# mandt-lab/PSLD

Hardware: AMD Instinct MI355X
Metric: train images/sec, CIFAR-10 PSLD (6ch 32x32) NCSN++ HSM step (higher is better)
Workload: dtype f32

## Files before the change

psld_amd/csrc/conv_wino.hip:

```cpp
#include <cstdlib>
#include <cstring>
#include <type_traits>

#include "common.h"
#include "psld_hip.h"
#include "tile_shared.h"
#include "limb.h"

namespace {

constexpr int WT = 32;
constexpr int VPLANE = WT * ROWB;
constexpr int VBYTES = 16 * 3 * VPLANE;
constexpr int WINO_THREADS = 512;

struct WinoArgs {
    const float* x1;
    const float* x2;
    int C1, C2;
    int B, H, W;
    const u32x4* ufrag;
    int N, M;
    int chunks;
    float* C;
// ... 111 lines not shown
        int lo = 0, hi = ntab - 1;
        while (lo < hi) {
            const int mid = (lo + hi + 1) >> 1;
            if (tab[8 * mid + 7] <= idx) lo = mid; else hi = mid - 1;
        }
        const long long* d = tab + 8 * lo;
        wino_pack_item<NL>(reinterpret_cast<const float*>(d[0]), reinterpret_cast<u32x4*>(d[1]), idx - d[7], (int)d[3], d[5], d[6],
                       (int)d[4]);
    }
}

template <int ABL = 0, bool GNF = false, bool ERAW = false, int LA = 2, bool TAIL = false, int NL = 3, bool SH = false>
__global__ void __launch_bounds__(WINO_THREADS) wino_conv8s_kernel(const WinoArgs a) {
    extern __shared__ __attribute__((aligned(16))) unsigned char smem[];
    constexpr int NI = 4;
    constexpr int RAWB = NI * 64 * 128;
    unsigned char* Vs = smem;
    unsigned char* Rs = smem + VBYTES / 3 * NL;

    const int tid = threadIdx.x;
    const int lane = tid & 63, wave = __builtin_amdgcn_readfirstlane(tid >> 6);
    const int tiles_n = TAIL ? (a.N + 127) >> 7 : a.N >> 7;
    const int nsp = a.ksplit > 1 ? a.ksplit : 1;
    const int tiles_m = a.tiles_m;
    const int per_range = tiles_m * tiles_n;
    const int vb = xcd_remap(blockIdx.x, gridDim.x);
    const int split = nsp > 1 ? vb / per_range : 0;
    const int bid = vb - split * per_range;
    const int kch = a.chunks >> a.lg_ksplit, ch0 = split * kch;
    float* const Cw = a.C + split * a.slab_stride;
    const int tile_n = a.nmajor ? bid / tiles_m : bid % tiles_n;
    const int tile_m = a.nmajor ? bid - tile_n * tiles_m : bid / tiles_n;
    const int n0 = tile_n * 128;
    const bool live = !TAIL || n0 + wave * 16 < a.N;

    const int HW = a.H * a.W;
    const int W2 = a.cw + 2;
    const int lg_tx = a.lg_tiles_x, lg_tps = a.lg_tps;
    const int rpi = HW >= 128 ? HW >> 7 : 1;
    const int tm_img = a.lg_rpi >= 0 ? tile_m >> a.lg_rpi : tile_m / rpi;
    const int reg = tile_m - tm_img * rpi;
    const int img0 = HW >= 128 ? tm_img : tile_m * a.nseg;
    const int oy0 = (reg >> a.lg_xblocks) * a.rps, ox0 = (reg & ((1 << a.lg_xblocks) - 1)) * a.cw;
    const float* zp = a.zero;

    const int c4 = tid & 7;
    int hoff[NI], rdst[NI];
    {
        const int seg_px = (a.rps + 2) * W2;
#pragma unroll
        for (int i = 0; i < NI; ++i) {
            const int px = (tid + WINO_THREADS * i) >> 3;
            const int seg = wino_div16(px, a.mul_seg);
            const int rem = px - seg * seg_px;
            const int hr = wino_div16(rem, a.mul_w2), hx = rem - hr * W2;
            const int img = img0 + seg, iy = oy0 + hr - 1, ix = ox0 + hx - 1;
            const bool ok = seg < a.nseg && img < a.B && iy >= 0 && iy < a.H && ix >= 0 && ix < a.W;
            hoff[i] = ok ? (img * a.H + iy) * a.W + ix : -1;
            rdst[i] = raw_off(px, c4);
        }
    }
    f32x4 hv[NI];
    auto load_raw = [&](int c) {
        const int c0 = c * 32;
        const bool second = c0 >= a.C1;
        const float* src = second ? a.x2 : a.x1;
        const int cs = second ? a.C2 : a.C1;
// ... 53 lines not shown
#pragma unroll
        for (int c = 0; c < 4; ++c) {
            ea[c] = *reinterpret_cast<const f32x4*>(Rb + t_ro[ra_ - v_r][c]);
            eb[c] = *reinterpret_cast<const f32x4*>(Rb + t_ro[rb_ - v_r][c]);
        }
        f32x4 r[4];
#pragma unroll
        for (int c = 0; c < 4; ++c) r[c] = plus ? ea[c] + eb[c] : ea[c] - eb[c];
#pragma unroll
        for (int j = 0; j < 4; ++j) {
            const f32x4 v = j == 0 ? r[0] - r[2] : j == 1 ? r[1] + r[2] : j == 2 ? r[2] - r[1] : r[1] - r[3];
            unsigned h0, m0_, l0, h1, m1, l1;
            if constexpr (NL == 3) {
                split3(v[0], v[1], h0, m0_, l0);
                split3(v[2], v[3], h1, m1, l1);
            } else if constexpr (NL == 2) {
                split2(v[0], v[1], h0, m0_);
                split2(v[2], v[3], h1, m1);
            } else if constexpr (SH) {
                h0 = cvt_pk_f16(v[0] * a.opscale, v[1] * a.opscale);
                h1 = cvt_pk_f16(v[2] * a.opscale, v[3] * a.opscale);
            } else {
                h0 = cvt_pk_f16(v[0], v[1]);
                h1 = cvt_pk_f16(v[2], v[3]);
            }
            unsigned char* q = Vs + (vrow * 4 + j) * NL * VPLANE + t_dst;
            *reinterpret_cast<u32x2*>(q) = u32x2{h0, h1};
            if constexpr (NL >= 2) *reinterpret_cast<u32x2*>(q + VPLANE) = u32x2{m0_, m1};
            if constexpr (NL == 3) *reinterpret_cast<u32x2*>(q + 2 * VPLANE) = u32x2{l0, l1};
        }
    };

    const int r16 = lane & 15, kq = lane >> 4;
    int aoff[2];
#pragma unroll
    for (int tb = 0; tb < 2; ++tb) {
        const int row = tb * 16 + r16;
        aoff[tb] = row * ROWB + ((kq ^ lds_swz(row)) << 4);
    }
    const u32x4* ub = a.ufrag + ((long long)(tile_n * 8 + ((ABL & 128) ? (wave & 3) : wave)) * a.chunks + ch0) * (16 * NL * 64);
    u32x4 bq[4][NL];
    auto load_b = [&](int sigma, u32x4 (&dst)[NL]) {
        const u32x4* p = ub + (long long)sigma * (NL * 64);
#pragma unroll
        for (int l = 0; l < NL; ++l) dst[l] = p[l * 64 + lane];
    };
    f32x4v acc[16][2];
#pragma unroll
    for (int p = 0; p < 16; ++p)
#pragma unroll
        for (int tb = 0; tb < 2; ++tb) acc[p][tb] = f32x4v{0.f, 0.f, 0.f, 0.f};
    u32x4 fa[NL == 1 ? 2 : NL][2];
    auto read_a = [&](int p, int l) {
#pragma unroll
        for (int tb = 0; tb < 2; ++tb) fa[l][tb] = *reinterpret_cast<const u32x4*>(Vs + (p * NL + l) * VPLANE + aoff[tb]);
    };
    auto mm = [&](int p, int la, int lb) {
#pragma unroll
        for (int tb = 0; tb < 2; ++tb) {
            if constexpr (NL == 1)
                acc[p][tb] = __builtin_amdgcn_mfma_f32_16x16x32_f16(
                    __builtin_bit_cast(f16x8, bq[p & 3][lb]), __builtin_bit_cast(f16x8, fa[la][tb]), acc[p][tb], 0, 0, 0);
            else
                acc[p][tb] = __builtin_amdgcn_mfma_f32_16x16x32_bf16(
                    __builtin_bit_cast(bf16x8, bq[p & 3][lb]), __builtin_bit_cast(bf16x8, fa[la][tb]), acc[p][tb], 0, 0, 0);
        }
    };
    auto mfma_half = [&](auto HH, auto LAST, int c) {
        constexpr int h = decltype(HH)::value;
        constexpr bool last = decltype(LAST)::value;
        if constexpr ((ABL & 256) != 0) __builtin_amdgcn_s_setprio(2);
        if constexpr (NL == 1) {
            auto read_a1 = [&](int p) {
#pragma unroll
                for (int tb = 0; tb < 2; ++tb) fa[p & 1][tb] = *reinterpret_cast<const u32x4*>(Vs + p * VPLANE + aoff[tb]);
            };
            read_a1(8 * h);
#pragma unroll
            for (int i = 0; i < 8; ++i) {
                const int p = 8 * h + i;
                if (!(last && p + LA >= 16)) load_b(c * 16 + p + LA, bq[(p + LA) & 3]);
                if (i < 7) read_a1(p + 1);
                __builtin_amdgcn_sched_barrier(0);
                mm(p, p & 1, 0);
                __builtin_amdgcn_sched_barrier(0);
            }
            return;
        }
        if constexpr (NL == 3) read_a(8 * h, 2);
        if constexpr (NL >= 2) read_a(8 * h, 1);
        read_a(8 * h, 0);
#pragma unroll
        for (int i = 0; i < 8; ++i) {
            const int p = 8 * h + i;
            if (!(ABL & 2) && !(last && p + LA >= 16)) load_b(c * 16 + p + LA, bq[(p + LA) & 3]);
            __builtin_amdgcn_sched_barrier(0);
            if constexpr (NL == 3) {
                mm(p, 2, 0);
                __builtin_amdgcn_sched_barrier(0);
                if (i < 7) read_a(p + 1, 2);
                __builtin_amdgcn_sched_barrier(0);
                mm(p, 1, 1);
            }
            if constexpr (NL >= 2) {
                mm(p, 1, 0);
                __builtin_amdgcn_sched_barrier(0);
                if (i < 7) read_a(p + 1, 1);
                __builtin_amdgcn_sched_barrier(0);
            }
            if constexpr (NL == 3) mm(p, 0, 2);
            if constexpr (NL >= 2) mm(p, 0, 1);
            mm(p, 0, 0);
            __builtin_amdgcn_sched_barrier(0);
            if (i < 7) read_a(p + 1, 0);
        }
        if constexpr ((ABL & 256) != 0) __builtin_amdgcn_s_setprio(0);
    };
    using I0 = std::integral_constant<int, 0>;
    using I1 = std::integral_constant<int, 1>;
    if constexpr ((ABL & 4) == 0 && (ABL & 256) == 0) { if (vr != 0) __builtin_amdgcn_s_setprio(1); }

    load_raw(ch0);
    if (live) {
        load_b(0, bq[0]);
        load_b(1, bq[1]);
        if (LA > 2) load_b(2, bq[2]);
    }
    store_raw(0, ch0);
    if constexpr (ERAW) load_raw(ch0 + min(1, kch - 1));
    __syncthreads();
    if (vr == 0) transform(I0{}, I0{}, 0); else transform(I0{}, I1{}, 0);
    __syncthreads();

    auto stamp = [&](int c, int idx) {
        if constexpr ((ABL & 64) != 0) {
            if (c == 3 && a.dbg) {
                __builtin_amdgcn_sched_barrier(0);
                const unsigned long long t = __builtin_amdgcn_s_memtime();
                if (lane == 0) a.dbg[((long long)blockIdx.x * 8 + wave) * 8 + idx] = t;
                __builtin_amdgcn_sched_barrier(0);
            }
        }
    };
    using No = std::false_type;
    using Yes = std::true_type;

    for (int c = 0; c < kch - 1; ++c) {
        stamp(c, 0);
        if constexpr (!ERAW) load_raw(ch0 + c + 1);
        if (vr == 0 && !(ABL & 1)) transform(I1{}, I0{}, c & 1);
        __builtin_amdgcn_sched_barrier(0);
        if (vr == 0) stamp(c, 1);
        if (live) mfma_half(I0{}, No{}, c);
        __builtin_amdgcn_sched_barrier(0);
        if (vr != 0) stamp(c, 1);
        if (vr != 0 && !(ABL & 1)) transform(I1{}, I1{}, c & 1);
        stamp(c, 2);
        store_raw((c + 1) & 1, ch0 + c + 1);
        stamp(c, 3);
// ... 4 lines not shown
        if (vr == 0) stamp(c, 5);
        if (live) mfma_half(I1{}, No{}, c);
        __builtin_amdgcn_sched_barrier(0);
        if (vr != 0) stamp(c, 5);
        if constexpr (ERAW) load_raw(ch0 + min(c + 2, kch - 1));
        if (vr != 0 && !(ABL & 1)) transform(I0{}, I1{}, (c + 1) & 1);
        stamp(c, 6);
        __syncthreads();
        stamp(c, 7);
    }
    {
        int c = kch - 1;
        asm volatile("" : "+s"(c));
        stamp(c, 0);
        if (vr == 0 && !(ABL & 1)) transform(I1{}, I0{}, c & 1);
        __builtin_amdgcn_sched_barrier(0);
        if (vr == 0) stamp(c, 1);
        if (live) mfma_half(I0{}, No{}, c);
        __builtin_amdgcn_sched_barrier(0);
        if (vr != 0) stamp(c, 1);
        if (vr != 0 && !(ABL & 1)) transform(I1{}, I1{}, c & 1);
        stamp(c, 2);
        stamp(c, 3);
        __syncthreads();
        stamp(c, 4);
        __builtin_amdgcn_sched_barrier(0);
        stamp(c, 5);
        if (live) mfma_half(I1{}, Yes{}, c);
        __builtin_amdgcn_sched_barrier(0);
        stamp(c, 6);
        stamp(c, 7);
    }

    if (!live) return;
    const PsldEpilogue& e = a.e;
    const int cn = n0 + wave * 16 + 4 * kq;
    const int org = (img0 * a.H + oy0) * a.W + ox0;
    const f32x4v zero4 = {0.f, 0.f, 0.f, 0.f};
    const bool rb_div = e.rowbias && !a.rb_img;
    char* const c_b = reinterpret_cast<char*>(Cw + (long long)org * a.ldc);
    const char* const res_b = reinterpret_cast<const char*>(e.res ? e.res + (long long)org * e.ldres : zp);
    f32x4v epi_bias, epi_tbv[2], epi_rv[2][4], epi_cv[2][4];
    int epi_rel[2];
    bool epi_ok[2];
    auto epi_rows = [&](auto TB) {
        constexpr int tb = decltype(TB)::value;
#pragma unroll
        for (int j = 0; j < 4; ++j) {
            const int px = epi_rel[tb] + (j >> 1) * a.W + (j & 1);
            epi_rv[tb][j] = e.res ? *reinterpret_cast<const f32x4v*>(res_b + (unsigned)((px * e.ldres + cn) * 4)) : zero4;
            epi_cv[tb][j] = e.accumulate ? *reinterpret_cast<const f32x4v*>(c_b + (unsigned)((px * a.ldc + cn) * 4)) : zero4;
        }
    };
    auto epi_request = [&]() {
        epi_bias = e.bias ? *reinterpret_cast<const f32x4v*>(e.bias + cn) : zero4;
#pragma unroll
        for (int tb = 0; tb < 2; ++tb) {
            const int tile = tb * 16 + r16;
            const int seg = tile >> lg_tps, rem = tile & ((1 << lg_tps) - 1);
            const int ty = rem >> lg_tx, tx = rem & ((1 << lg_tx) - 1);
            epi_ok[tb] = img0 + seg < a.B;
            epi_rel[tb] = epi_ok[tb] ? seg * HW + 2 * ty * a.W + 2 * tx : 0;
            epi_tbv[tb] = a.rb_img ? *reinterpret_cast<const f32x4v*>(
                                         e.rowbias + (long long)(epi_ok[tb] ? img0 + seg : img0) * e.ld_rowbias + cn)
                                   : zero4;
        }
        epi_rows(I0{});
    };
    epi_request();
    epi_rows(I1{});
    const f32x4v bias4 = epi_bias;
#pragma unroll
    for (int tb = 0; tb < 2; ++tb) {
        const bool ok = epi_ok[tb];
        const int rel = epi_rel[tb];
#pragma unroll
        for (int i = 0; i < 4; ++i) {
            const f32x4v s0 = (acc[4 * i][tb] + acc[4 * i + 1][tb]) + acc[4 * i + 2][tb];
            acc[4 * i + 1][tb] = (acc[4 * i + 1][tb] - acc[4 * i + 2][tb]) - acc[4 * i + 3][tb];
            acc[4 * i][tb] = s0;
        }
        const f32x4v add4 = bias4 + epi_tbv[tb];
        f32x4v o[2][2];
#pragma unroll
        for (int ya = 0; ya < 2; ++ya)
#pragma unroll
            for (int xb = 0; xb < 2; ++xb) {
                const f32x4v y = ya == 0 ? (acc[xb][tb] + acc[4 + xb][tb]) + acc[8 + xb][tb]
                                         : (acc[4 + xb][tb] - acc[8 + xb][tb]) - acc[12 + xb][tb];
                f32x4v addv = add4;
                if (rb_div)
                    addv = bias4 + *reinterpret_cast<const f32x4v*>(
                                       e.rowbias + (long long)((org + rel + ya * a.W + xb) / e.rows_per_img) * e.ld_rowbias + cn);
                f32x4v x = y * e.alpha + addv;
                if (e.res) x += epi_rv[tb][ya * 2 + xb];
                x *= e.out_scale;
                if (e.accumulate) x += epi_cv[tb][ya * 2 + xb];
                o[ya][xb] = x;
            }
        const bool gn_on = e.gn_part != nullptr;
        double gs = 0.0, gss = 0.0;
        if (ok) {
#pragma unroll
            for (int ya = 0; ya < 2; ++ya)
#pragma unroll
                for (int xb = 0; xb < 2; ++xb) {
                    const int px = rel + ya * a.W + xb;
                    if ((ABL & 8) && org + px != 0) continue;
                    *reinterpret_cast<f32x4v*>(c_b + (unsigned)((px * a.ldc + cn) * 4)) = o[ya][xb];
                    if (gn_on) {
#pragma unroll
                        for (int v = 0; v < 4; ++v) {
                            const double d = (double)o[ya][xb][v];
                            gs += d;
                            gss = fma(d, d, gss);
                        }
                    }
                }
        }
        if (gn_on) {
            double s1 = gs, s2 = gss;
#pragma unroll
            for (int sft = 1; sft <= 8; sft <<= 1) {
                s1 += __shfl_xor(s1, sft, 64);
                s2 += __shfl_xor(s2, sft, 64);
            }
            const double q1 = s1, q2 = s2;
            s1 += __shfl_xor(s1, 16, 64);
            s2 += __shfl_xor(s2, 16, 64);
            const int img = a.nseg == 1 ? img0 : img0 + tb, chunk = a.nseg == 1 ? 2 * reg + tb : 0, chunks = e.gn_hw >> 6;
            if (e.gn_fine == 4) {
                if ((lane & 0xf) == 0 && img < a.B) {
                    const int f = ((n0 + wave * 16) >> 2) + (lane >> 4);
                    double* pp = e.gn_part + (((long long)img * chunks + chunk) * (a.N >> 2) + f) * 2;
                    pp[0] = q1;
                    pp[1] = q2;
                }
            } else if ((lane & 0x1f) == 0 && img < a.B) {
                const int f = ((n0 + wave * 16) >> 3) + (lane >> 5);
                double* pp = e.gn_part + (((long long)img * chunks + chunk) * (a.N >> 3) + f) * 2;
                pp[0] = s1;
                pp[1] = s2;
            }
        }
    }
}

#ifdef PSLD_ABLATIONS
#include "conv_wino_abl.inc"
#endif

template <int ABL = 0, bool GNF = false, bool ERAW = false, int LA = 2, bool TAIL = false, int NL = 3, bool SH = false>
int launch_wino8s(const WinoArgs& a, hipStream_t stream, const char* name) {
    constexpr size_t LDS = (size_t)VBYTES / 3 * NL + 2 * (size_t)4 * 64 * 128;
    static_assert(LDS <= 163840, "LDS budget");
    if (int st = psld_lds_once<&wino_conv8s_kernel<ABL, GNF, ERAW, LA, TAIL, NL, SH>>(LDS, name)) return st;
    PSLD_CHECK_ARG(a.tiles_m == cdiv(a.M, 128) && (1 << a.lg_ksplit) == (a.ksplit > 1 ? a.ksplit : 1),
                   "%s: launch geometry not filled in (tiles_m %d, ksplit %d)", name, a.tiles_m, a.ksplit);
    dim3 grid((unsigned)(a.tiles_m * cdiv(a.N, 128) * (a.ksplit > 1 ? a.ksplit : 1)));
    hipLaunchKernelGGL((wino_conv8s_kernel<ABL, GNF, ERAW, LA, TAIL, NL, SH>), grid, dim3(WINO_THREADS), LDS, stream, a);
    PSLD_CHECK_LAUNCH(name);
    return PSLD_OK;
}

int wino_cu_count() {
    static int n[PSLD_MAX_DEVICES] = {};
    int& cu = n[psld_device_slot()];
    if (cu <= 0) {
        int dev = 0;
        if (hipGetDevice(&dev) != hipSuccess || hipDeviceGetAttribute(&cu, hipDeviceAttributeMultiprocessorCount, dev) != hipSuccess ||
            cu <= 0)
            cu = 256;
// ... 339 lines not shown
```

psld_amd/csrc/pointwise.hip:

```cpp
#include "common.h"
#include "psld_hip.h"

namespace {

inline int grid_for(long long n, int per_thread = 1) {
    long long b = (n + 256LL * per_thread - 1) / (256LL * per_thread);
    if (b > 256LL * 16) b = 256LL * 16;
    if (b < 1) b = 1;
    return (int)b;
}

#define GRID_STRIDE(i, n) \
    for (long long i = (long long)blockIdx.x * blockDim.x + threadIdx.x; i < (n); i += (long long)gridDim.x * blockDim.x)

__global__ void transpose_kernel(const float* __restrict__ x, float* __restrict__ y, int rows, int cols) {
    __shared__ float tile[32][33];
    const long long img = blockIdx.z;
    const float* xp = x + img * rows * cols;
    float* yp = y + img * rows * cols;
    const int c0 = blockIdx.x * 32, r0 = blockIdx.y * 32;
    const int tx = threadIdx.x & 31, ty = threadIdx.x >> 5;
    for (int j = ty; j < 32; j += 8) {
        const int r = r0 + j, c = c0 + tx;
        if (r < rows && c < cols) tile[j][tx] = xp[(long long)r * cols + c];
// ... 347 lines not shown
#pragma unroll
                    for (int p = 0; p < 4; ++p) {
                        const f32x4 xv = win[ky][p + kx];
                        float a = acc[p][o];
                        a = fmaf(xv[0], wv[0], a);
                        a = fmaf(xv[1], wv[1], a);
                        a = fmaf(xv[2], wv[2], a);
                        a = fmaf(xv[3], wv[3], a);
                        acc[p][o] = a;
                    }
                }
            }
        }
#pragma unroll
        for (int p = 0; p < 4; ++p)
#pragma unroll
            for (int o = 0; o < COUT; ++o) {
                float v = acc[p][o];
#pragma unroll
                for (int sft = 32; sft >= 1; sft >>= 1) v += __shfl_xor(v, sft, 64);
                acc[p][o] = v;
            }
        if (lane < 4 && ox0 + lane < w) {
            float* yo = y + (((n * h + oy) * w + ox0 + lane) * COUT);
#pragma unroll
            for (int o = 0; o < COUT; ++o) {
                float v = lane == 0 ? acc[0][o] : lane == 1 ? acc[1][o] : lane == 2 ? acc[2][o] : acc[3][o];
                yo[o] = v + (bias ? bias[o] : 0.f);
            }
        }
    }
}

__global__ void copy_batch_kernel(const long long* __restrict__ tab, int ntab, long long total4) {
    GRID_STRIDE(i, total4) {
        int lo = 0, hi = ntab - 1;
        while (lo < hi) {
            const int mid = (lo + hi + 1) >> 1;
            if (tab[4 * mid + 3] <= i) lo = mid; else hi = mid - 1;
        }
        const long long* d = tab + 4 * lo;
        const long long j = i - d[3];
        reinterpret_cast<f32x4*>(d[1])[j] = reinterpret_cast<const f32x4*>(d[0])[j];
    }
}

__global__ void scale_copy2d_kernel(const float* __restrict__ src, int ld_src, float* __restrict__ dst, int ld_dst,
                                    long long rows, int cols, float alpha) {
    GRID_STRIDE(i, rows * cols) {
        const long long r = i / cols;
        const int j = (int)(i - r * cols);
        dst[r * ld_dst + j] = alpha * src[r * ld_src + j];
    }
}

__global__ void axpby_kernel(const float* __restrict__ a, float sa, const float* __restrict__ b, float sb,
                             float* __restrict__ y, long long n4, long long n, int accumulate) {
    GRID_STRIDE(i, n4) {
        f32x4 v = reinterpret_cast<const f32x4*>(a)[i] * sa;
        if (b) v += reinterpret_cast<const f32x4*>(b)[i] * sb;
        if (accumulate) v += reinterpret_cast<const f32x4*>(y)[i];
        reinterpret_cast<f32x4*>(y)[i] = v;
    }
    const long long t0 = n4 * 4;
    GRID_STRIDE(j, n - t0) {
        const long long i = t0 + j;
// ... 80 lines not shown
        for (int l = 0; l < 64; ++l) t += red[l][cl];
        const float v = (float)(t * (double)alpha);
        if (seg <= 0 || col < seg) out[col] = v;
        else if (col < 2 * seg) out1[col - seg] = v;
        else out2[col - 2 * seg] = v;
    }
}
__global__ void colsum_kernel(const float* __restrict__ x, int ld, int hw, int c, float* __restrict__ out,
                              float alpha) {
    __shared__ double red[4][64];
    const int b = blockIdx.y;
    const int col = blockIdx.x * 64 + (threadIdx.x & 63);
    const int rl = threadIdx.x >> 6;
    double acc = 0.0;
    if (col < c) {
        const float* p = x + ((long long)b * hw) * ld + col;
        float part = 0.f;
        int cnt = 0;
        for (int r = rl; r < hw; r += 4) {
            part += p[(long long)r * ld];
            if (++cnt == 32) {
                acc += (double)part;
                part = 0.f;
                cnt = 0;
            }
        }
        acc += (double)part;
    }
    red[rl][threadIdx.x & 63] = acc;
    __syncthreads();
    if (rl == 0 && col < c) out[(long long)b * c + col] = (float)((red[0][threadIdx.x] + red[1][threadIdx.x] + red[2][threadIdx.x] + red[3][threadIdx.x]) * (double)alpha);
}

template <int V>
__global__ void softmax_rows_reg_kernel(const float* __restrict__ x, float* __restrict__ y, long long rows, int L) {
    const long long row = (long long)blockIdx.x * (blockDim.x >> 6) + (threadIdx.x >> 6);
    if (row >= rows) return;
    const int lane = threadIdx.x & 63;
    const f32x4* xp = reinterpret_cast<const f32x4*>(x + row * L);
    f32x4 v[V];
    float mx = -INFINITY;
#pragma unroll
    for (int j = 0; j < V; ++j) {
        v[j] = xp[lane + 64 * j];
        mx = fmaxf(mx, fmaxf(fmaxf(v[j][0], v[j][1]), fmaxf(v[j][2], v[j][3])));
    }
    mx = wave_max(mx);
    float s = 0.f;
#pragma unroll
    for (int j = 0; j < V; ++j)
#pragma unroll
        for (int e = 0; e < 4; ++e) {
            v[j][e] = expf(v[j][e] - mx);
            s += v[j][e];
        }
    s = wave_sum(s);
    const float inv = 1.0f / s;
    f32x4* yp = reinterpret_cast<f32x4*>(y + row * L);
#pragma unroll
    for (int j = 0; j < V; ++j) yp[lane + 64 * j] = v[j] * inv;
}
template <int V>
__global__ void softmax_rows_bwd_reg_kernel(const float* __restrict__ y, const float* __restrict__ dy,
                                            float* __restrict__ dx, long long rows, int L) {
    const long long row = (long long)blockIdx.x * (blockDim.x >> 6) + (threadIdx.x >> 6);
    if (row >= rows) return;
// ... 203 lines not shown
                                  float* cols, hipStream_t stream) {
    PSLD_CHECK_ARG(x && cols && batch > 0 && c > 0 && c % 4 == 0 && oh > 0 && ow > 0 && stride >= 1 && pad >= 0 &&
                       (reinterpret_cast<uintptr_t>(x) & 15) == 0 && (reinterpret_cast<uintptr_t>(cols) & 15) == 0,
                   "psld_im2col3x3_f32: bad args (c=%d)", c);
    const long long total4 = (long long)batch * oh * ow * 9 * (c / 4);
    hipLaunchKernelGGL(im2col3x3_kernel, dim3(grid_for(total4)), dim3(256), 0, stream, x, ih, iw, c / 4, oh, ow, stride, pad,
                       cols, total4);
    PSLD_CHECK_LAUNCH("psld_im2col3x3_f32");
    return PSLD_OK;
}

extern "C" int psld_col2im3x3_f32(const float* dcols, int batch, int ih, int iw, int c, int oh, int ow, int stride, int pad,
                                  float* dx, hipStream_t stream) {
    PSLD_CHECK_ARG(dcols && dx && batch > 0 && c > 0 && c % 4 == 0 && oh > 0 && ow > 0 && stride >= 1 && pad >= 0 &&
                       (reinterpret_cast<uintptr_t>(dx) & 15) == 0 && (reinterpret_cast<uintptr_t>(dcols) & 15) == 0,
                   "psld_col2im3x3_f32: bad args (c=%d)", c);
    const long long total4 = (long long)batch * ih * iw * (c / 4);
    hipLaunchKernelGGL(col2im3x3_kernel, dim3(grid_for(total4)), dim3(256), 0, stream, dcols, ih, iw, c / 4, oh, ow, stride,
                       pad, dx, total4);
    PSLD_CHECK_LAUNCH("psld_col2im3x3_f32");
    return PSLD_OK;
}

extern "C" int psld_conv3x3_fewout_supported(int cin, int cout) {
    return cin > 0 && cin % 4 == 0 && cin <= 256 && (cout == 3 || cout == 6) && 9 * cout * cin * 4 <= 64 * 1024;
}

extern "C" int psld_conv3x3_fewout_f32(const float* x, const float* w_ohwi, const float* bias, float* y, int batch,
                                       int h, int w, int cin, int cout, hipStream_t stream) {
    PSLD_CHECK_ARG(x && w_ohwi && y && batch > 0 && h > 0 && w > 0, "psld_conv3x3_fewout_f32: bad args");
    PSLD_CHECK_ARG(psld_conv3x3_fewout_supported(cin, cout), "psld_conv3x3_fewout_f32: unsupported cin=%d cout=%d", cin, cout);
    PSLD_CHECK_ARG((reinterpret_cast<uintptr_t>(x) & 15) == 0, "psld_conv3x3_fewout_f32: unaligned input");
    const size_t lds = (size_t)9 * cout * cin * sizeof(float);
    const long long groups = (long long)batch * h * ((w + 3) / 4);
    long long blocks = (groups + 3) / 4;
    if (blocks > 2048) blocks = 2048;
    if (cout == 6) {
        static PsldPerDeviceFlag configured_; bool& configured = configured_.here();
        if (!configured) {
            (void)hipFuncSetAttribute(reinterpret_cast<const void*>(&conv3x3_fewout_kernel<6>),
                                      hipFuncAttributeMaxDynamicSharedMemorySize, 64 * 1024);
            configured = true;
        }
        hipLaunchKernelGGL(conv3x3_fewout_kernel<6>, dim3((unsigned)blocks), dim3(256), lds, stream, x, w_ohwi, bias, y, batch,
                           h, w, cin);
    } else {
        static PsldPerDeviceFlag configured_; bool& configured = configured_.here();
        if (!configured) {
            (void)hipFuncSetAttribute(reinterpret_cast<const void*>(&conv3x3_fewout_kernel<3>),
                                      hipFuncAttributeMaxDynamicSharedMemorySize, 64 * 1024);
            configured = true;
        }
        hipLaunchKernelGGL(conv3x3_fewout_kernel<3>, dim3((unsigned)blocks), dim3(256), lds, stream, x, w_ohwi, bias, y, batch,
                           h, w, cin);
    }
    PSLD_CHECK_LAUNCH("psld_conv3x3_fewout_f32");
    return PSLD_OK;
}

extern "C" int psld_copy_batch_f32(const long long* table_dev, int entries, long long total4, hipStream_t stream) {
    PSLD_CHECK_ARG(table_dev && entries > 0 && total4 > 0, "psld_copy_batch_f32: bad args");
    hipLaunchKernelGGL(copy_batch_kernel, dim3(grid_for(total4)), dim3(256), 0, stream, table_dev, entries, total4);
    PSLD_CHECK_LAUNCH("psld_copy_batch_f32");
    return PSLD_OK;
}

// ... 41 lines not shown
    hipLaunchKernelGGL(silu_bwd_kernel, dim3(grid_for(n)), dim3(256), 0, stream, x, dy, dx, n);
    PSLD_CHECK_LAUNCH("psld_silu_bwd_f32");
    return PSLD_OK;
}
extern "C" long long psld_colsum_workspace_bytes(int batch, int hw, int c) {
    return (long long)batch * 64 * c * sizeof(double) + 256;
}
extern "C" int psld_colsum_f32(const float* x, int ld, int batch, int hw, int c, float* out, float alpha,
                               void* workspace, hipStream_t stream) {
    PSLD_CHECK_ARG(x && out && batch > 0 && hw > 0 && c > 0, "psld_colsum_f32: bad args");
    const bool vec = workspace && c % 4 == 0 && ld % 4 == 0 && c / 4 <= 256 && hw >= 8 &&
                     (reinterpret_cast<uintptr_t>(x) & 15) == 0;
    if (vec) {
        const int cq = c / 4;
        int pl = 256 / cq;
        if (pl < 1) pl = 1;
        if (pl > hw) pl = hw;
        int chunks = cdiv(1024, batch);
        const int max_chunks = cdiv(hw, pl * 4);
        if (chunks > max_chunks) chunks = max_chunks;
        if (chunks > 16) chunks = 16;
        if (chunks < 1) chunks = 1;
        const int chunk_px = cdiv(hw, chunks);
        chunks = cdiv(hw, chunk_px);
        double* part = reinterpret_cast<double*>(workspace);
        hipLaunchKernelGGL(colsum_partial_kernel, dim3(chunks, batch), dim3(cq * pl), (size_t)pl * cq * 4 * sizeof(double),
                           stream, x, ld, hw, c, cq, pl, chunk_px, chunks, part);
        PSLD_CHECK_LAUNCH("colsum_partial_kernel");
        hipLaunchKernelGGL(colsum_final_kernel, dim3(cdiv(c, 128), batch), dim3(128), 0, stream, part, chunks, c, out,
                           alpha, c);
        PSLD_CHECK_LAUNCH("colsum_final_kernel");
        return PSLD_OK;
    }
    hipLaunchKernelGGL(colsum_kernel, dim3(cdiv(c, 64), batch), dim3(256), 0, stream, x, ld, hw, c, out, alpha);
    PSLD_CHECK_LAUNCH("psld_colsum_f32");
    return PSLD_OK;
}
extern "C" int psld_bias_grad_f32(const float* x, int ld, int batch, int hw, int c, float* per_image, int ld_per_image,
                                  float* out, float alpha, void* workspace, hipStream_t stream) {
    PSLD_CHECK_ARG(x && out && workspace && batch > 0 && hw > 0 && c > 0, "psld_bias_grad_f32: bad args");
    PSLD_CHECK_ARG(c % 4 == 0 && ld % 4 == 0 && c / 4 <= 256 && (reinterpret_cast<uintptr_t>(x) & 15) == 0,
                   "psld_bias_grad_f32: needs c %%4 == 0 (<= 1024), ld %%4 == 0 and a 16-byte aligned input");
    const int cq = c / 4;
    int pl = 256 / cq;
    if (pl < 1) pl = 1;
    if (pl > hw) pl = hw;
    int chunks = cdiv(1024, batch);
    const int max_chunks = cdiv(hw, pl * 4);
    if (chunks > max_chunks) chunks = max_chunks;
    if (chunks > 16) chunks = 16;
    if (chunks < 1) chunks = 1;
    const int chunk_px = cdiv(hw, chunks);
    chunks = cdiv(hw, chunk_px);
    double* part = reinterpret_cast<double*>(workspace);
    float* pim = per_image ? per_image : reinterpret_cast<float*>(part + (long long)batch * 16 * c);
    const int ldp = per_image && ld_per_image > 0 ? ld_per_image : c;
    hipLaunchKernelGGL(colsum_partial_kernel, dim3(chunks, batch), dim3(cq * pl), (size_t)pl * cq * 4 * sizeof(double),
                       stream, x, ld, hw, c, cq, pl, chunk_px, chunks, part);
    PSLD_CHECK_LAUNCH("colsum_partial_kernel");
    hipLaunchKernelGGL(colsum_final_total_kernel, dim3(cdiv(c, 16)), dim3(1024), 0, stream, part, chunks, batch, c, pim, ldp,
                       out, alpha);
    PSLD_CHECK_LAUNCH("colsum_final_total_kernel");
    return PSLD_OK;
}
extern "C" int psld_bias_grad_seg_f32(const float* x, int ld, int batch, int hw, int seg, float* out0, float* out1,
                                      float* out2, float alpha, void* workspace, hipStream_t stream) {
    const int c = 3 * seg;
// ... 136 lines not shown
```

Before: 1255.

## Split Winograd GEMM across waves by transform-plane halves with LDS accumulator exchange

```diff
diff --git a/psld_amd/csrc/conv_wino.hip b/psld_amd/csrc/conv_wino.hip
--- a/psld_amd/csrc/conv_wino.hip
+++ b/psld_amd/csrc/conv_wino.hip
@@ -167,7 +167,7 @@
     const int tile_n = a.nmajor ? bid / tiles_m : bid % tiles_n;
     const int tile_m = a.nmajor ? bid - tile_n * tiles_m : bid / tiles_n;
     const int n0 = tile_n * 128;
-    const bool live = !TAIL || n0 + wave * 16 < a.N;
+    const bool live = !TAIL || n0 + (wave & 3) * 32 < a.N;
 
     const int HW = a.H * a.W;
     const int W2 = a.cw + 2;
@@ -287,87 +287,99 @@
     };
 
     const int r16 = lane & 15, kq = lane >> 4;
+    const int g = wave & 3;
     int aoff[2];
 #pragma unroll
     for (int tb = 0; tb < 2; ++tb) {
-        const int row = tb * 16 + r16;
-        aoff[tb] = row * ROWB + ((kq ^ lds_swz(row)) << 4);
-    }
-    const u32x4* ub = a.ufrag + ((long long)(tile_n * 8 + ((ABL & 128) ? (wave & 3) : wave)) * a.chunks + ch0) * (16 * NL * 64);
+        const int row = (tb ^ vr) * 16 + r16;
+        aoff[tb] = row * ROWB + ((kq ^ lds_swz(row)) << 4) + vr * (4 * NL * VPLANE);
+    }
+    const u32x4* ub[2];
+#pragma unroll
+    for (int cb = 0; cb < 2; ++cb)
+        ub[cb] = a.ufrag + ((long long)(tile_n * 8 + 2 * g + cb) * a.chunks + ch0) * (16 * NL * 64) + vr * (4 * NL * 64);
     u32x4 bq[4][NL];
-    auto load_b = [&](int sigma, u32x4 (&dst)[NL]) {
-        const u32x4* p = ub + (long long)sigma * (NL * 64);
+    auto load_b = [&](int sigma, int cb, u32x4 (&dst)[NL]) {
+        const u32x4* p = ub[cb] + (long long)sigma * (NL * 64);
 #pragma unroll
         for (int l = 0; l < NL; ++l) dst[l] = p[l * 64 + lane];
     };
-    f32x4v acc[16][2];
-#pragma unroll
-    for (int p = 0; p < 16; ++p)
-#pragma unroll
-        for (int tb = 0; tb < 2; ++tb) acc[p][tb] = f32x4v{0.f, 0.f, 0.f, 0.f};
+    f32x4v acc[8][2][2];
+#pragma unroll
+    for (int q = 0; q < 8; ++q)
+#pragma unroll
+        for (int cb = 0; cb < 2; ++cb)
+#pragma unroll
+            for (int tb = 0; tb < 2; ++tb) acc[q][cb][tb] = f32x4v{0.f, 0.f, 0.f, 0.f};
     u32x4 fa[NL == 1 ? 2 : NL][2];
-    auto read_a = [&](int p, int l) {
-#pragma unroll
-        for (int tb = 0; tb < 2; ++tb) fa[l][tb] = *reinterpret_cast<const u32x4*>(Vs + (p * NL + l) * VPLANE + aoff[tb]);
+    auto read_a = [&](int pl, int l) {
+#pragma unroll
+        for (int tb = 0; tb < 2; ++tb) fa[l][tb] = *reinterpret_cast<const u32x4*>(Vs + (pl * NL + l) * VPLANE + aoff[tb]);
     };
-    auto mm = [&](int p, int la, int lb) {
+    auto mm = [&](int q, int cb, int slot, int la, int lb) {
 #pragma unroll
         for (int tb = 0; tb < 2; ++tb) {
             if constexpr (NL == 1)
-                acc[p][tb] = __builtin_amdgcn_mfma_f32_16x16x32_f16(
-                    __builtin_bit_cast(f16x8, bq[p & 3][lb]), __builtin_bit_cast(f16x8, fa[la][tb]), acc[p][tb], 0, 0, 0);
+                acc[q][cb][tb] = __builtin_amdgcn_mfma_f32_16x16x32_f16(
+                    __builtin_bit_cast(f16x8, bq[slot][lb]), __builtin_bit_cast(f16x8, fa[la][tb]), acc[q][cb][tb], 0, 0, 0);
             else
-                acc[p][tb] = __builtin_amdgcn_mfma_f32_16x16x32_bf16(
-                    __builtin_bit_cast(bf16x8, bq[p & 3][lb]), __builtin_bit_cast(bf16x8, fa[la][tb]), acc[p][tb], 0, 0, 0);
+                acc[q][cb][tb] = __builtin_amdgcn_mfma_f32_16x16x32_bf16(
+                    __builtin_bit_cast(bf16x8, bq[slot][lb]), __builtin_bit_cast(bf16x8, fa[la][tb]), acc[q][cb][tb], 0, 0, 0);
         }
     };
     auto mfma_half = [&](auto HH, auto LAST, int c) {
-        constexpr int h = decltype(HH)::value;
+        constexpr int th = decltype(HH)::value;
         constexpr bool last = decltype(LAST)::value;
         if constexpr ((ABL & 256) != 0) __builtin_amdgcn_s_setprio(2);
+        auto ahead = [&](int u) {
+            const int v = u + LA;
+            if (!(ABL & 2) && !(last && v >= 8)) load_b(c * 16 + 8 * th + ((v >> 1) & 3) + 8 * (v >> 3), v & 1, bq[v & 3]);
+        };
         if constexpr (NL == 1) {
-            auto read_a1 = [&](int p) {
-#pragma unroll
-                for (int tb = 0; tb < 2; ++tb) fa[p & 1][tb] = *reinterpret_cast<const u32x4*>(Vs + p * VPLANE + aoff[tb]);
+            auto read_a1 = [&](int j) {
+#pragma unroll
+                for (int tb = 0; tb < 2; ++tb)
+                    fa[j & 1][tb] = *reinterpret_cast<const u32x4*>(Vs + (8 * th + j) * VPLANE + aoff[tb]);
             };
-            read_a1(8 * h);
-#pragma unroll
-            for (int i = 0; i < 8; ++i) {
-                const int p = 8 * h + i;
-                if (!(last && p + LA >= 16)) load_b(c * 16 + p + LA, bq[(p + LA) & 3]);
-                if (i < 7) read_a1(p + 1);
+            read_a1(0);
+#pragma unroll
+            for (int u = 0; u < 8; ++u) {
+                const int j = u >> 1, cb = u & 1;
+                ahead(u);
+                if (cb == 0 && j < 3) read_a1(j + 1);
                 __builtin_amdgcn_sched_barrier(0);
-                mm(p, p & 1, 0);
+                mm(4 * th + j, cb, u & 3, j & 1, 0);
                 __builtin_amdgcn_sched_barrier(0);
             }
             return;
         }
-        if constexpr (NL == 3) read_a(8 * h, 2);
-        if constexpr (NL >= 2) read_a(8 * h, 1);
-        read_a(8 * h, 0);
-#pragma unroll
-        for (int i = 0; i < 8; ++i) {
-            const int p = 8 * h + i;
-            if (!(ABL & 2) && !(last && p + LA >= 16)) load_b(c * 16 + p + LA, bq[(p + LA) & 3]);
+        if constexpr (NL == 3) read_a(8 * th, 2);
+        if constexpr (NL >= 2) read_a(8 * th, 1);
+        read_a(8 * th, 0);
+#pragma unroll
+        for (int u = 0; u < 8; ++u) {
+            const int j = u >> 1, cb = u & 1, q = 4 * th + j;
+            ahead(u);
             __builtin_amdgcn_sched_barrier(0);
+            const bool rd = cb == 1 && j < 3;
             if constexpr (NL == 3) {
-                mm(p, 2, 0);
+                mm(q, cb, u & 3, 2, 0);
                 __builtin_amdgcn_sched_barrier(0);
-                if (i < 7) read_a(p + 1, 2);
+                if (rd) read_a(8 * th + j + 1, 2);
                 __builtin_amdgcn_sched_barrier(0);
-                mm(p, 1, 1);
+                mm(q, cb, u & 3, 1, 1);
             }
             if constexpr (NL >= 2) {
-                mm(p, 1, 0);
+                mm(q, cb, u & 3, 1, 0);
                 __builtin_amdgcn_sched_barrier(0);
-                if (i < 7) read_a(p + 1, 1);
+                if (rd) read_a(8 * th + j + 1, 1);
                 __builtin_amdgcn_sched_barrier(0);
             }
-            if constexpr (NL == 3) mm(p, 0, 2);
-            if constexpr (NL >= 2) mm(p, 0, 1);
-            mm(p, 0, 0);
+            if constexpr (NL == 3) mm(q, cb, u & 3, 0, 2);
+            if constexpr (NL >= 2) mm(q, cb, u & 3, 0, 1);
+            mm(q, cb, u & 3, 0, 0);
             __builtin_amdgcn_sched_barrier(0);
-            if (i < 7) read_a(p + 1, 0);
+            if (rd) read_a(8 * th + j + 1, 0);
         }
         if constexpr ((ABL & 256) != 0) __builtin_amdgcn_s_setprio(0);
     };
@@ -377,9 +389,9 @@
 
     load_raw(ch0);
     if (live) {
-        load_b(0, bq[0]);
-        load_b(1, bq[1]);
-        if (LA > 2) load_b(2, bq[2]);
+        load_b(0, 0, bq[0]);
+        load_b(0, 1, bq[1]);
+        if (LA > 2) load_b(1, 0, bq[2]);
     }
     store_raw(0, ch0);
     if constexpr (ERAW) load_raw(ch0 + min(1, kch - 1));
@@ -450,70 +462,91 @@
         stamp(c, 7);
     }
 
-    if (!live) return;
     const PsldEpilogue& e = a.e;
-    const int cn = n0 + wave * 16 + 4 * kq;
+    const int el = __builtin_amdgcn_mbcnt_hi(~0u, __builtin_amdgcn_mbcnt_lo(~0u, 0u)), er16 = el & 15, ekq = el >> 4;
+    const int cn0 = n0 + g * 32 + 4 * ekq;
     const int org = (img0 * a.H + oy0) * a.W + ox0;
     const f32x4v zero4 = {0.f, 0.f, 0.f, 0.f};
     const bool rb_div = e.rowbias && !a.rb_img;
     char* const c_b = reinterpret_cast<char*>(Cw + (long long)org * a.ldc);
     const char* const res_b = reinterpret_cast<const char*>(e.res ? e.res + (long long)org * e.ldres : zp);
-    f32x4v epi_bias, epi_tbv[2], epi_rv[2][4], epi_cv[2][4];
-    int epi_rel[2];
-    bool epi_ok[2];
-    auto epi_rows = [&](auto TB) {
-        constexpr int tb = decltype(TB)::value;
-#pragma unroll
-        for (int j = 0; j < 4; ++j) {
-            const int px = epi_rel[tb] + (j >> 1) * a.W + (j & 1);
-            epi_rv[tb][j] = e.res ? *reinterpret_cast<const f32x4v*>(res_b + (unsigned)((px * e.ldres + cn) * 4)) : zero4;
-            epi_cv[tb][j] = e.accumulate ? *reinterpret_cast<const f32x4v*>(c_b + (unsigned)((px * a.ldc + cn) * 4)) : zero4;
-        }
-    };
-    auto epi_request = [&]() {
-        epi_bias = e.bias ? *reinterpret_cast<const f32x4v*>(e.bias + cn) : zero4;
-#pragma unroll
-        for (int tb = 0; tb < 2; ++tb) {
-            const int tile = tb * 16 + r16;
-            const int seg = tile >> lg_tps, rem = tile & ((1 << lg_tps) - 1);
-            const int ty = rem >> lg_tx, tx = rem & ((1 << lg_tx) - 1);
-            epi_ok[tb] = img0 + seg < a.B;
-            epi_rel[tb] = epi_ok[tb] ? seg * HW + 2 * ty * a.W + 2 * tx : 0;
-            epi_tbv[tb] = a.rb_img ? *reinterpret_cast<const f32x4v*>(
-                                         e.rowbias + (long long)(epi_ok[tb] ? img0 + seg : img0) * e.ld_rowbias + cn)
+    f32x4v epi_bias[2], epi_tbv[2], epi_rv[2][4], epi_cv[2][4];
+    bool ok = false;
+    int rel = 0;
+    if (live) {
+        const int tile = vr * 16 + er16;
+        const int seg = tile >> lg_tps, rem = tile & ((1 << lg_tps) - 1);
+        const int ty = rem >> lg_tx, tx = rem & ((1 << lg_tx) - 1);
+        ok = img0 + seg < a.B;
+        rel = ok ? seg * HW + 2 * ty * a.W + 2 * tx : 0;
+#pragma unroll
+        for (int cb = 0; cb < 2; ++cb) {
+            const int cn = cn0 + 16 * cb;
+            epi_bias[cb] = e.bias ? *reinterpret_cast<const f32x4v*>(e.bias + cn) : zero4;
+            epi_tbv[cb] = a.rb_img ? *reinterpret_cast<const f32x4v*>(e.rowbias + (long long)(ok ? img0 + seg : img0) * e.ld_rowbias + cn)
                                    : zero4;
         }
-        epi_rows(I0{});
-    };
-    epi_request();
-    epi_rows(I1{});
-    const f32x4v bias4 = epi_bias;
-#pragma unroll
-    for (int tb = 0; tb < 2; ++tb) {
-        const bool ok = epi_ok[tb];
-        const int rel = epi_rel[tb];
-#pragma unroll
-        for (int i = 0; i < 4; ++i) {
-            const f32x4v s0 = (acc[4 * i][tb] + acc[4 * i + 1][tb]) + acc[4 * i + 2][tb];
-            acc[4 * i + 1][tb] = (acc[4 * i + 1][tb] - acc[4 * i + 2][tb]) - acc[4 * i + 3][tb];
-            acc[4 * i][tb] = s0;
-        }
-        const f32x4v add4 = bias4 + epi_tbv[tb];
+#pragma unroll
+        for (int cb = 0; cb < 2; ++cb)
+#pragma unroll
+            for (int j = 0; j < 4; ++j) {
+                const int px = rel + (j >> 1) * a.W + (j & 1), cn = cn0 + 16 * cb;
+                epi_rv[cb][j] = e.res ? *reinterpret_cast<const f32x4v*>(res_b + (unsigned)((px * e.ldres + cn) * 4)) : zero4;
+                epi_cv[cb][j] = e.accumulate ? *reinterpret_cast<const f32x4v*>(c_b + (unsigned)((px * a.ldc + cn) * 4)) : zero4;
+            }
+#pragma unroll
+        for (int th = 0; th < 2; ++th)
+#pragma unroll
+            for (int cb = 0; cb < 2; ++cb)
+#pragma unroll
+                for (int tb = 0; tb < 2; ++tb) {
+                    const f32x4v s0 = (acc[4 * th][cb][tb] + acc[4 * th + 1][cb][tb]) + acc[4 * th + 2][cb][tb];
+                    acc[4 * th + 1][cb][tb] = (acc[4 * th + 1][cb][tb] - acc[4 * th + 2][cb][tb]) - acc[4 * th + 3][cb][tb];
+                    acc[4 * th][cb][tb] = s0;
+                }
+        unsigned char* const xs = Rs + (wave * 8 * 64 + el) * 16;
+#pragma unroll
+        for (int th = 0; th < 2; ++th)
+#pragma unroll
+            for (int xb = 0; xb < 2; ++xb)
+#pragma unroll
+                for (int cb = 0; cb < 2; ++cb)
+                    *reinterpret_cast<f32x4v*>(xs + ((th * 2 + xb) * 2 + cb) * 1024) = acc[4 * th + xb][cb][1];
+    }
+    __syncthreads();
+    if (!live) return;
+    {
+        const unsigned char* const xr = Rs + ((wave ^ 4) * 8 * 64 + el) * 16;
+#pragma unroll
+        for (int th = 0; th < 2; ++th)
+#pragma unroll
+            for (int xb = 0; xb < 2; ++xb)
+#pragma unroll
+                for (int cb = 0; cb < 2; ++cb)
+                    acc[4 * th + xb][cb][1] = *reinterpret_cast<const f32x4v*>(xr + ((th * 2 + xb) * 2 + cb) * 1024);
+    }
+    const bool odd = vr != 0;
+#pragma unroll
+    for (int cb = 0; cb < 2; ++cb) {
+        const int cn = cn0 + 16 * cb;
+        const f32x4v bias4 = epi_bias[cb];
+        const f32x4v add4 = bias4 + epi_tbv[cb];
         f32x4v o[2][2];
 #pragma unroll
         for (int ya = 0; ya < 2; ++ya)
 #pragma unroll
             for (int xb = 0; xb < 2; ++xb) {
-                const f32x4v y = ya == 0 ? (acc[xb][tb] + acc[4 + xb][tb]) + acc[8 + xb][tb]
-                                         : (acc[4 + xb][tb] - acc[8 + xb][tb]) - acc[12 + xb][tb];
+                const f32x4v r0 = odd ? acc[xb][cb][1] : acc[xb][cb][0], r1 = odd ? acc[xb][cb][0] : acc[xb][cb][1];
+                const f32x4v r2 = odd ? acc[4 + xb][cb][1] : acc[4 + xb][cb][0], r3 = odd ? acc[4 + xb][cb][0] : acc[4 + xb][cb][1];
+                const f32x4v y = ya == 0 ? (r0 + r1) + r2 : (r1 - r2) - r3;
                 f32x4v addv = add4;
                 if (rb_div)
                     addv = bias4 + *reinterpret_cast<const f32x4v*>(
                                        e.rowbias + (long long)((org + rel + ya * a.W + xb) / e.rows_per_img) * e.ld_rowbias + cn);
                 f32x4v x = y * e.alpha + addv;
-                if (e.res) x += epi_rv[tb][ya * 2 + xb];
+                if (e.res) x += epi_rv[cb][ya * 2 + xb];
                 x *= e.out_scale;
-                if (e.accumulate) x += epi_cv[tb][ya * 2 + xb];
+                if (e.accumulate) x += epi_cv[cb][ya * 2 + xb];
                 o[ya][xb] = x;
             }
         const bool gn_on = e.gn_part != nullptr;
@@ -546,16 +579,16 @@
             const double q1 = s1, q2 = s2;
             s1 += __shfl_xor(s1, 16, 64);
             s2 += __shfl_xor(s2, 16, 64);
-            const int img = a.nseg == 1 ? img0 : img0 + tb, chunk = a.nseg == 1 ? 2 * reg + tb : 0, chunks = e.gn_hw >> 6;
+            const int img = a.nseg == 1 ? img0 : img0 + vr, chunk = a.nseg == 1 ? 2 * reg + vr : 0, chunks = e.gn_hw >> 6;
             if (e.gn_fine == 4) {
-                if ((lane & 0xf) == 0 && img < a.B) {
-                    const int f = ((n0 + wave * 16) >> 2) + (lane >> 4);
+                if ((el & 0xf) == 0 && img < a.B) {
+                    const int f = ((n0 + g * 32 + cb * 16) >> 2) + (el >> 4);
                     double* pp = e.gn_part + (((long long)img * chunks + chunk) * (a.N >> 2) + f) * 2;
                     pp[0] = q1;
                     pp[1] = q2;
                 }
-            } else if ((lane & 0x1f) == 0 && img < a.B) {
-                const int f = ((n0 + wave * 16) >> 3) + (lane >> 5);
+            } else if ((el & 0x1f) == 0 && img < a.B) {
+                const int f = ((n0 + g * 32 + cb * 16) >> 3) + (el >> 5);
                 double* pp = e.gn_part + (((long long)img * chunks + chunk) * (a.N >> 3) + f) * 2;
                 pp[0] = s1;
                 pp[1] = s2;
```

New measurement: 1272, median of 6. 1.01x the previous value.

## Add streaming few-output 3x3 conv kernel and small-channel colsum kernel

Applied to the files above, without the earlier changes.

```diff
diff --git a/psld_amd/csrc/pointwise.hip b/psld_amd/csrc/pointwise.hip
--- a/psld_amd/csrc/pointwise.hip
+++ b/psld_amd/csrc/pointwise.hip
@@ -403,6 +403,98 @@
     }
 }
 
+constexpr int FEWOUT_PX = 8;
+template <int V, int OFF, int N>
+__device__ __forceinline__ void fold_lanes(float (&a)[N], int lane, int& first) {
+    if constexpr (OFF > 0) {
+        if constexpr (V % 2 == 0) {
+            constexpr int H = V / 2;
+            const bool up = (lane & OFF) != 0;
+#pragma unroll
+            for (int i = 0; i < H; ++i) {
+                const float send = up ? a[i] : a[i + H];
+                const float keep = up ? a[i + H] : a[i];
+                a[i] = keep + __shfl_xor(send, OFF, 64);
+            }
+            if (up) first += H;
+            fold_lanes<H, OFF / 2>(a, lane, first);
+        } else {
+#pragma unroll
+            for (int i = 0; i < V; ++i) a[i] += __shfl_xor(a[i], OFF, 64);
+            fold_lanes<V, OFF / 2>(a, lane, first);
+        }
+    }
+}
+constexpr int fold_count(int v, int off) { return off == 0 ? v : fold_count(v % 2 == 0 ? v / 2 : v, off / 2); }
+constexpr int fold_dup(int v, int off) { return off == 0 ? 0 : ((v % 2 ? off : 0) | fold_dup(v % 2 == 0 ? v / 2 : v, off / 2)); }
+
+template <int COUT, int LS>
+__global__ void __launch_bounds__(256) conv3x3_fewout_stream_kernel(const float* __restrict__ x, const float* __restrict__ w_ohwi,
+                                                                   const float* __restrict__ bias, float* __restrict__ y,
+                                                                   int batch, int h, int w) {
+    constexpr int C = 4 * LS, SLOTS = 256 / LS, V = FEWOUT_PX * COUT;
+    extern __shared__ __attribute__((aligned(16))) float wl[];
+    for (int i = threadIdx.x; i < 9 * COUT * C; i += 256) {
+        const int ch = i % C, r = i / C;
+        const int o = r % COUT, t = r / COUT;
+        wl[i] = w_ohwi[((long long)o * 9 + t) * C + ch];
+    }
+    __syncthreads();
+    const int l = threadIdx.x % LS, slot = threadIdx.x / LS;
+    const unsigned runs = (unsigned)(w + FEWOUT_PX - 1) / FEWOUT_PX;
+    const unsigned total = (unsigned)batch * h * runs;
+    const f32x4* x4 = reinterpret_cast<const f32x4*>(x);
+    for (unsigned base = blockIdx.x * SLOTS; base < total; base += gridDim.x * SLOTS) {
+        const unsigned s = base + slot;
+        const bool live = s < total;
+        const unsigned row = (live ? s : 0u) / runs;
+        const int ox0 = (int)((live ? s : 0u) - row * runs) * FEWOUT_PX;
+        const long long n = row / (unsigned)h;
+        const int oy = (int)(row - (unsigned)n * h);
+        float acc[V];
+#pragma unroll
+        for (int i = 0; i < V; ++i) acc[i] = 0.f;
+#pragma unroll 1
+        for (int ky = 0; ky < 3; ++ky) {
+            const int iy = oy + ky - 1;
+            const bool rowok = live && iy >= 0 && iy < h;
+            f32x4 xr[FEWOUT_PX + 2];
+#pragma unroll
+            for (int d = 0; d < FEWOUT_PX + 2; ++d) {
+                const int ix = ox0 + d - 1;
+                xr[d] = (rowok && ix >= 0 && ix < w) ? x4[((n * h + iy) * w + ix) * LS + l] : f32x4{0.f, 0.f, 0.f, 0.f};
+            }
+#pragma unroll
+            for (int kx = 0; kx < 3; ++kx)
+#pragma unroll
+                for (int o = 0; o < COUT; ++o) {
+                    const f32x4 wv = *reinterpret_cast<const f32x4*>(wl + ((ky * 3 + kx) * COUT + o) * C + l * 4);
+#pragma unroll
+                    for (int p = 0; p < FEWOUT_PX; ++p) {
+                        const f32x4 xv = xr[p + kx];
+                        float a = acc[p * COUT + o];
+                        a = fmaf(xv[0], wv[0], a);
+                        a = fmaf(xv[1], wv[1], a);
+                        a = fmaf(xv[2], wv[2], a);
+                        a = fmaf(xv[3], wv[3], a);
+                        acc[p * COUT + o] = a;
+                    }
+                }
+        }
+        int first = 0;
+        fold_lanes<V, LS / 2>(acc, l, first);
+        constexpr int VF = fold_count(V, LS / 2), DUP = fold_dup(V, LS / 2);
+        if (live && (l & DUP) == 0) {
+            float* yo = y + ((n * h + oy) * w + ox0) * COUT;
+#pragma unroll
+            for (int i = 0; i < VF; ++i) {
+                const int v = first + i, p = v / COUT, o = v - p * COUT;
+                if (ox0 + p < w) yo[v] = acc[i] + (bias ? bias[o] : 0.f);
+            }
+        }
+    }
+}
+
 __global__ void copy_batch_kernel(const long long* __restrict__ tab, int ntab, long long total4) {
     GRID_STRIDE(i, total4) {
         int lo = 0, hi = ntab - 1;
@@ -549,6 +641,36 @@
     if (rl == 0 && col < c) out[(long long)b * c + col] = (float)((red[0][threadIdx.x] + red[1][threadIdx.x] + red[2][threadIdx.x] + red[3][threadIdx.x]) * (double)alpha);
 }
 
+__global__ void __launch_bounds__(256) colsum_few_kernel(const float* __restrict__ x, int ld, int hw, int c,
+                                                         float* __restrict__ out, float alpha) {
+    extern __shared__ float part[];
+    __shared__ double red[4][16];
+    const int b = blockIdx.x;
+    const int groups = ((hw + 3) / 4 + 31) / 32;
+    const float* p = x + (long long)b * hw * ld;
+    for (int u = threadIdx.x; u < groups * 4 * c; u += 256) {
+        const int col = u % c, rl = (u / c) & 3, g = u / (4 * c);
+        float s = 0.f;
+#pragma unroll 8
+        for (int k = 0; k < 32; ++k) {
+            const int r = rl + 4 * (g * 32 + k);
+            if (r < hw) s += p[(long long)r * ld + col];
+        }
+        part[u] = s;
+    }
+    __syncthreads();
+    if (threadIdx.x < 4 * c) {
+        const int col = threadIdx.x % c, rl = threadIdx.x / c;
+        double acc = 0.0;
+        for (int g = 0; g < groups; ++g) acc += (double)part[(g * 4 + rl) * c + col];
+        red[rl][col] = acc;
+    }
+    __syncthreads();
+    if (threadIdx.x < c)
+        out[(long long)b * c + threadIdx.x] =
+            (float)((red[0][threadIdx.x] + red[1][threadIdx.x] + red[2][threadIdx.x] + red[3][threadIdx.x]) * (double)alpha);
+}
+
 template <int V>
 __global__ void softmax_rows_reg_kernel(const float* __restrict__ x, float* __restrict__ y, long long rows, int L) {
     const long long row = (long long)blockIdx.x * (blockDim.x >> 6) + (threadIdx.x >> 6);
@@ -818,6 +940,24 @@
     PSLD_CHECK_ARG(psld_conv3x3_fewout_supported(cin, cout), "psld_conv3x3_fewout_f32: unsupported cin=%d cout=%d", cin, cout);
     PSLD_CHECK_ARG((reinterpret_cast<uintptr_t>(x) & 15) == 0, "psld_conv3x3_fewout_f32: unaligned input");
     const size_t lds = (size_t)9 * cout * cin * sizeof(float);
+    const long long runs = (long long)batch * h * ((w + FEWOUT_PX - 1) / FEWOUT_PX);
+    if ((cin == 128 || cin == 256) && runs < (1ll << 31)) {
+        const unsigned grid = psld_grid_blocks(runs, 1024 / cin, 512);
+#define PSLD_FEWOUT_STREAM(COUT, LS)                                                                                        \
+    do {                                                                                                                    \
+        const int st = psld_lds_once<conv3x3_fewout_stream_kernel<COUT, LS>>(lds, "psld_conv3x3_fewout_f32");               \
+        if (st != PSLD_OK) return st;                                                                                       \
+        hipLaunchKernelGGL((conv3x3_fewout_stream_kernel<COUT, LS>), dim3(grid), dim3(256), lds, stream, x, w_ohwi, bias,  \
+                           y, batch, h, w);                                                                                 \
+    } while (0)
+        if (cout == 6 && cin == 128) PSLD_FEWOUT_STREAM(6, 32);
+        else if (cout == 6) PSLD_FEWOUT_STREAM(6, 64);
+        else if (cin == 128) PSLD_FEWOUT_STREAM(3, 32);
+        else PSLD_FEWOUT_STREAM(3, 64);
+#undef PSLD_FEWOUT_STREAM
+        PSLD_CHECK_LAUNCH("psld_conv3x3_fewout_f32");
+        return PSLD_OK;
+    }
     const long long groups = (long long)batch * h * ((w + 3) / 4);
     long long blocks = (groups + 3) / 4;
     if (blocks > 2048) blocks = 2048;
@@ -925,7 +1065,12 @@
         PSLD_CHECK_LAUNCH("colsum_final_kernel");
         return PSLD_OK;
     }
-    hipLaunchKernelGGL(colsum_kernel, dim3(cdiv(c, 64), batch), dim3(256), 0, stream, x, ld, hw, c, out, alpha);
+    const int groups = ((hw + 3) / 4 + 31) / 32;
+    const size_t few_lds = (size_t)groups * 4 * c * sizeof(float);
+    if (c <= 16 && groups >= 2 && few_lds <= 48 * 1024)
+        hipLaunchKernelGGL(colsum_few_kernel, dim3(batch), dim3(256), few_lds, stream, x, ld, hw, c, out, alpha);
+    else
+        hipLaunchKernelGGL(colsum_kernel, dim3(cdiv(c, 64), batch), dim3(256), 0, stream, x, ld, hw, c, out, alpha);
     PSLD_CHECK_LAUNCH("psld_colsum_f32");
     return PSLD_OK;
 }
```

Measured after the change: 1282 before, 1287 after (median of 6 runs). About the same (+0.3%).
